# skypilot-org/skypilot

Hardware: AMD Instinct MI355X
Metric: tokens/sec (node) sky-launched Llama-3-8B (higher is better)
Workload: dtype bf16; 1 GPU; model=llama3-8b, global_batch=6, seq_len=4096, parallelism=dp1, sky_launched=True

## Files before the change

### skypilot_amd/models/llama.py

```python
from __future__ import annotations

import math
from dataclasses import dataclass

import torch
import torch.nn as nn

from skypilot_amd import ops


@dataclass
class LlamaConfig:
    name: str = "llama3-8b"
    vocab_size: int = 128256
    hidden_size: int = 4096
    intermediate_size: int = 14336
    num_layers: int = 32
    num_heads: int = 32
    num_kv_heads: int = 8
    head_dim: int = 128
    rope_theta: float = 500000.0
    norm_eps: float = 1e-5
    max_seq_len: int = 8192
    tie_embeddings: bool = False
# ... 51 lines not shown
                                      i32(lens))
        cache.write_rows_fp8(attn.layer_idx, k, v, *infer_ctx.kv_write_idx)
        return
    for i, (slot, ln) in enumerate(zip(slots, lens)):
        cache.write_prefill(attn.layer_idx, slot, k[i:i + 1], v[i:i + 1], ln)


def append_attention(attn, q, k, v, infer_ctx):
    cache = infer_ctx.cache
    if cache.kv_dtype == "fp8":
        li = attn.layer_idx
        cache.write_rows_fp8(li, k, v, infer_ctx.append_slots,
                             infer_ctx.append_start, infer_ctx.append_lens)
        return ops.attn_append_fp8(q, cache.k[li], cache.v[li],
                                   cache.k_exp[li], cache.v_exp[li],
                                   infer_ctx.append_slots,
                                   infer_ctx.append_start,
                                   infer_ctx.append_lens, attn.scale)
    for i, (slot, start, ln) in enumerate(zip(infer_ctx.append_slots_l,
                                              infer_ctx.append_start_l,
                                              infer_ctx.append_lens_l)):
        cache.write_append(attn.layer_idx, slot, start, k[i:i + 1],
                           v[i:i + 1], ln)
    return ops.attn_append(q, cache.k[attn.layer_idx],
                           cache.v[attn.layer_idx], infer_ctx.append_slots,
                           infer_ctx.append_start, infer_ctx.append_lens,
                           attn.scale)


class Attention(nn.Module):
    def __init__(self, cfg: LlamaConfig):
        super().__init__()
        self.cfg = cfg
        h, d = cfg.hidden_size, cfg.head_dim
        self.n_q, self.n_kv = cfg.num_heads, cfg.num_kv_heads
        self.wq = nn.Linear(h, self.n_q * d, bias=cfg.attn_bias)
        self.wk = nn.Linear(h, self.n_kv * d, bias=cfg.attn_bias)
        self.wv = nn.Linear(h, self.n_kv * d, bias=cfg.attn_bias)
        self.wo = nn.Linear(self.n_q * d, h, bias=False)
        self.scale = 1.0 / math.sqrt(d)
        self._wqkv = None
        self._bqkv = None

    def packed_qkv(self):
        if self._wqkv is None:
            self._wqkv = torch.cat(
                [self.wq.weight, self.wk.weight, self.wv.weight],
                0).contiguous()
            if self.wq.bias is not None:
                self._bqkv = torch.cat(
                    [self.wq.bias, self.wk.bias, self.wv.bias],
                    0).contiguous()
        return self._wqkv

    def forward(self, x, cos, sin, positions, infer_ctx=None,
                qkv=None):
        d = self.cfg.head_dim
        if x is None:
            B, S = qkv.shape[0], 1
        else:
            B, S, _ = x.shape
        decode = infer_ctx is not None and infer_ctx.mode == "decode"
        if decode:
            cache = infer_ctx.cache
            if qkv is None:
                qkv = ops.decode_linear(x.reshape(B, -1),
                                        self.packed_qkv())
            qkv = qkv.reshape(B, -1)
            if self._bqkv is not None:
                qkv = qkv + self._bqkv
            li = self.layer_idx
            if cache.kv_dtype == "fp8":
                o = ops.attn_decode_qkv_fp8(
                    qkv, cache.k[li], cache.v[li], cache.k_exp[li],
                    cache.v_exp[li], cos, sin, positions, infer_ctx.kv_lens,
                    infer_ctx.slot_ids_i32, self.n_q, self.n_kv, self.scale)
            else:
                o = ops.attn_decode_qkv(
                    qkv, cache.k[li], cache.v[li], cos, sin, positions,
                    infer_ctx.kv_lens, infer_ctx.slot_ids_i32, self.n_q,
                    self.n_kv, self.scale)
            return ops.decode_linear(o.reshape(B, self.n_q * d),
                                     self.wo.weight).view(B, S, -1)
        lin = torch.nn.functional.linear
        q = lin(x, self.wq.weight, self.wq.bias).view(B, S, self.n_q, d)
        k = lin(x, self.wk.weight, self.wk.bias).view(B, S, self.n_kv, d)
        v = lin(x, self.wv.weight, self.wv.bias).view(B, S, self.n_kv, d)
        q = ops.rope(q.reshape(B * S, self.n_q, d), cos, sin,
                     positions).view(B, S, self.n_q, d)
        k = ops.rope(k.reshape(B * S, self.n_kv, d), cos, sin,
                     positions).view(B, S, self.n_kv, d)
        if infer_ctx is None:
            o = ops.attention(q, k, v, self.scale, causal=True)
        elif infer_ctx.mode == "append":
            o = append_attention(self, q, k, v, infer_ctx)
        else:
            prefill_cache_write(self, k, v, infer_ctx)
            o = ops.attention(q, k, v, self.scale, causal=True)
        return lin(o.reshape(B, S, self.n_q * d), self.wo.weight)


class MLP(nn.Module):
    def __init__(self, cfg: LlamaConfig):
        super().__init__()
        h, m = cfg.hidden_size, cfg.intermediate_size
        self.w_gate_up = nn.Linear(h, 2 * m, bias=False)
        self.w_down = nn.Linear(m, h, bias=False)
        self.m = m

    def forward(self, x, infer_ctx=None):
        decode = infer_ctx is not None and infer_ctx.mode == "decode"
        lin = ops.decode_linear if decode else torch.nn.functional.linear
        return lin(ops.swiglu(lin(x, self.w_gate_up.weight)),
                   self.w_down.weight)

    def down_from_gu(self, gu):
        return ops.decode_linear(ops.swiglu(gu), self.w_down.weight)



class Block(nn.Module):
    def __init__(self, cfg: LlamaConfig, layer_idx: int):
        super().__init__()
        self.attn = Attention(cfg)
        self.attn.layer_idx = layer_idx
        self.mlp = MLP(cfg)
        self.attn_norm = nn.Parameter(torch.ones(cfg.hidden_size))
        self.mlp_norm = nn.Parameter(torch.ones(cfg.hidden_size))
        self.eps = cfg.norm_eps

    def forward(self, x, cos, sin, positions, infer_ctx=None):
        x = x + self.attn(ops.rmsnorm(x, self.attn_norm, self.eps), cos, sin,
                          positions, infer_ctx)
        x = x + self.mlp(ops.rmsnorm(x, self.mlp_norm, self.eps),
                         infer_ctx)
        return x


class Llama(nn.Module):
    def __init__(self, cfg: LlamaConfig):
        super().__init__()
        self.cfg = cfg
        self.embed = nn.Embedding(cfg.vocab_size, cfg.hidden_size)
        self.blocks = nn.ModuleList(
            Block(cfg, i) for i in range(cfg.num_layers))
        self.final_norm = nn.Parameter(torch.ones(cfg.hidden_size))
        self.lm_head = nn.Linear(cfg.hidden_size, cfg.vocab_size, bias=False)
        if cfg.tie_embeddings:
            self.lm_head.weight = self.embed.weight
        self._rope = None

    def _tables(self, device):
        if self._rope is None or self._rope[0].device != device:
            self._rope = rope_tables(self.cfg, device)
        return self._rope

    def forward(self, tokens: torch.Tensor, positions: torch.Tensor = None,
                infer_ctx=None) -> torch.Tensor:
        B, S = tokens.shape
        cos, sin = self._tables(tokens.device)
        if positions is None:
            positions = torch.arange(S, dtype=torch.int32,
                                     device=tokens.device)
            positions = positions.unsqueeze(0).expand(B, S).reshape(-1)
        x = self.embed(tokens)
        if infer_ctx is not None and infer_ctx.mode == "decode":
            res = None
            for blk in self.blocks:
                if not hasattr(blk.attn, "_wqkv"):
                    if res is None:
                        h = ops.rmsnorm(x, blk.attn_norm, blk.eps)
                    else:
                        x, h = ops.rmsnorm_res(x, res, blk.attn_norm,
                                               blk.eps)
                    a = blk.attn(h, cos, sin, positions, infer_ctx)
                    x, h2 = ops.rmsnorm_res(x, a, blk.mlp_norm, blk.eps)
                    res = blk.mlp(h2, infer_ctx)
                    continue
                x, qkv = ops.decode_norm_linear(
                    x, res, blk.attn_norm, blk.eps, blk.attn.packed_qkv())
                a = blk.attn(None, cos, sin, positions, infer_ctx,
                             qkv=qkv)
                x, gu = ops.decode_norm_linear(
                    x, a, blk.mlp_norm, blk.eps, blk.mlp.w_gate_up.weight)
                res = blk.mlp.down_from_gu(gu)
            _, logits = ops.decode_norm_linear(
                x, res, self.final_norm, self.cfg.norm_eps,
                self.lm_head.weight)
            return logits
        for blk in self.blocks:
            x = blk(x, cos, sin, positions, infer_ctx)
        if infer_ctx is not None and infer_ctx.mode == "append":
            last = (infer_ctx.append_lens.long() - 1).clamp(min=0)
            x = x[torch.arange(B, device=x.device), last].unsqueeze(1)
        x = ops.rmsnorm(x, self.final_norm, self.cfg.norm_eps)
# ... 29 lines not shown
```

### skypilot_amd/ops/__init__.py

```python
from __future__ import annotations

import importlib.util
import math
import os
from pathlib import Path

import torch

_C = None
_LOAD_ERR: Exception | None = None


def _load():
    global _C, _LOAD_ERR
    if _C is not None:
        return _C
    so = Path(__file__).resolve().parent / "_C.so"
    try:
        if not so.exists():
            raise ImportError(
                f"native extension {so} not built; run "
                "`python -m skypilot_amd.ops.build`")
        spec = importlib.util.spec_from_file_location("skypilot_amd.ops._C",
                                                      so)
# ... 162 lines not shown
        with torch.enable_grad():
            qd = q.detach().requires_grad_()
            kd = k.detach().requires_grad_()
            vd = v.detach().requires_grad_()
            out = attention_ref(qd, kd, vd, ctx.scale, ctx.causal)
            gq, gk, gv = torch.autograd.grad(out, (qd, kd, vd), dO)
        return gq, gk, gv, None, None


def attention(q, k, v, scale=None, causal=True):
    if scale is None:
        scale = 1.0 / math.sqrt(q.shape[-1])
    return _AttentionFn.apply(q, k, v, scale, causal)


class _CrossEntropyFn(torch.autograd.Function):

    @staticmethod
    def forward(ctx, logits, targets, ignore_index):
        if logits.is_cuda:
            C = _require_native("cross_entropy")
            n_valid = int((targets != ignore_index).sum().item())
            n_valid = max(n_valid, 1)
            logits = logits.contiguous()
            loss = C.cross_entropy_fused(logits, targets.int(),
                                         1.0 / n_valid, ignore_index)
            ctx.save_for_backward(logits)
            ctx.native = True
            return loss.sum() / n_valid
        ctx.native = False
        ctx.save_for_backward(logits, targets)
        ctx.ignore_index = ignore_index
        return cross_entropy_ref(logits, targets, ignore_index)

    @staticmethod
    def backward(ctx, g):
        if ctx.native:
            (dlogits,) = ctx.saved_tensors
            if not (isinstance(g, torch.Tensor) and g.numel() == 1
                    and float(g) == 1.0):
                dlogits = dlogits * g
            return dlogits, None, None
        logits, targets = ctx.saved_tensors
        with torch.enable_grad():
            ld = logits.detach().requires_grad_()
            loss = cross_entropy_ref(ld, targets, ctx.ignore_index)
            (gl,) = torch.autograd.grad(loss, (ld,), g)
        return gl, None, None


def fused_cross_entropy(logits, targets, ignore_index: int = -100):
    return _CrossEntropyFn.apply(logits, targets, ignore_index)


class _SwiGLUFn(torch.autograd.Function):
    @staticmethod
    def forward(ctx, gu):
        ctx.save_for_backward(gu)
        if gu.is_cuda:
            C = _require_native("swiglu")
            return C.swiglu_fwd(gu.contiguous())
        M = gu.shape[-1] // 2
        g, u = gu.float().split(M, dim=-1)
        return (torch.nn.functional.silu(g) * u).to(gu.dtype)

    @staticmethod
    def backward(ctx, dy):
        (gu,) = ctx.saved_tensors
        if gu.is_cuda:
            C = native()
            return C.swiglu_bwd(gu.contiguous(), dy.contiguous())
        M = gu.shape[-1] // 2
        g, u = gu.float().split(M, dim=-1)
        dyf = dy.float()
        sg = torch.sigmoid(g)
        silu = g * sg
        dg = dyf * u * (sg + silu * (1 - sg))
        du = dyf * silu
        return torch.cat([dg, du], dim=-1).to(gu.dtype)


def swiglu(gu):
    return _SwiGLUFn.apply(gu)


def attn_decode_ref(q, kc, vc, kv_lens, slot_ids, scale):
    B, Hq, D = q.shape
    Hkv = kc.shape[2]
    rep = Hq // Hkv
    out = torch.empty_like(q)
    for i in range(B):
        slot = int(slot_ids[i])
        L = int(kv_lens[i])
        k = kc[slot, :L].float()
        v = vc[slot, :L].float()
        kf = k.repeat_interleave(rep, dim=1)
        vf = v.repeat_interleave(rep, dim=1)
        att = torch.einsum("hd,lhd->hl", q[i].float(), kf) * scale
        p = att.softmax(-1)
        out[i] = torch.einsum("hl,lhd->hd", p, vf).to(q.dtype)
    return out


def attn_decode(q, kc, vc, kv_lens, slot_ids, scale):
    if q.is_cuda:
        C = _require_native("attn_decode")
        return C.attn_decode(q.contiguous(), kc, vc, kv_lens.int(),
                             slot_ids.int(), scale)
    return attn_decode_ref(q, kc, vc, kv_lens, slot_ids, scale)


def attn_append_ref(q, kc, vc, slot_ids, q_start, q_lens, scale):
    n, Sq, Hq, D = q.shape
    S_max, Hkv = kc.shape[1], kc.shape[2]
    rep = Hq // Hkv
    out = torch.zeros_like(q)
    for b in range(n):
        slot, start, ln = int(slot_ids[b]), int(q_start[b]), int(q_lens[b])
        if ln == 0:
            continue
        L = min(start + ln, S_max)
        qf = q[b, :ln].float().permute(1, 0, 2)
        kf = kc[slot, :L].float().permute(1, 0, 2).repeat_interleave(
            rep, dim=0)
        vf = vc[slot, :L].float().permute(1, 0, 2).repeat_interleave(
            rep, dim=0)
        att = torch.matmul(qf, kf.transpose(-1, -2)) * scale
        pos = start + torch.arange(ln, device=q.device)
        mask = torch.arange(L, device=q.device)[None, :] > pos[:, None]
        p = att.masked_fill(mask, float("-inf")).softmax(-1)
        out[b, :ln] = torch.matmul(p, vf).permute(1, 0, 2).to(q.dtype)
    return out


def attn_append(q, kc, vc, slot_ids, q_start, q_lens, scale):
    if q.is_cuda:
        C = _require_native("attn_append")
        return C.attn_append(q.contiguous(), kc, vc, slot_ids, q_start,
                             q_lens, scale)
    return attn_append_ref(q, kc, vc, slot_ids, q_start, q_lens, scale)


def kv_quantize(x: torch.Tensor):
    xf = x.detach().float()
    amax = xf.abs().amax(-1)
    u = amax.contiguous().view(torch.int32) & 0x7FFFFFFF
    n = (u >> 23) - 135 + ((u & 0x7FFFFF) > 0x600000).to(torch.int32)
    n = n.clamp(-126, 127)
    n = torch.where(u == 0, torch.zeros_like(n), n)
    inv = ((127 - n).clamp(min=1) << 23).view(torch.float32)
    codes = (xf * inv.unsqueeze(-1)).to(torch.float8_e4m3fn).view(torch.uint8)
    return codes.contiguous(), (n + 127).to(torch.uint8)


def kv_dequantize(codes: torch.Tensor, exp: torch.Tensor) -> torch.Tensor:
    scale = (exp.to(torch.int32) << 23).view(torch.float32)
    return codes.view(torch.float8_e4m3fn).float() * scale.unsqueeze(-1)


def kv_write_fp8(k, v, kc, vc, ke, ve, slot_ids, starts, lens):
    if k.is_cuda:
        C = _require_native("kv_write_fp8")
        C.kv_write_fp8(k.contiguous(), v.contiguous(), kc, vc, ke, ve,
                       slot_ids, starts, lens)
        return
    n, S = k.shape[0], k.shape[1]
# ... 248 lines not shown
    blk = torch.empty(6, n, dtype=torch.int32)
    blk[0] = rowvec(temperature, torch.float32).contiguous().view(torch.int32)
    blk[1] = rowvec(top_p, torch.float32).contiguous().view(torch.int32)
    blk[2] = rowvec(clamp_k(top_k), torch.int64).clamp(
        0, 2 ** 31 - 1).to(torch.int32)
    blk[3] = (sd & _M32).to(torch.int32)
    blk[4] = (sd >> 32).to(torch.int32)
    blk[5] = rowvec(wrap32(counter), torch.int64).to(torch.int32)
    return blk


def sample_tokens_reference(logits, temperature, top_p, top_k, seed,
                            counter):
    logits = logits.reshape(-1, logits.shape[-1])
    n = logits.shape[0]
    blk = pack_samp(n, temperature, top_p, top_k, seed, counter)
    Ts = blk[0].view(torch.float32).tolist()
    ps = blk[1].view(torch.float32).tolist()
    ks = blk[2].tolist()
    los, his, cs = blk[3].tolist(), blk[4].tolist(), blk[5].tolist()
    toks, taus = [], []
    for i in range(n):
        sd = ((his[i] & _M32) << 32) | (los[i] & _M32)
        r = sample_row_reference(logits[i], Ts[i], ps[i], ks[i], sd, cs[i])
        toks.append(r["token"])
        taus.append(r["tau"])
    return (torch.tensor(toks, dtype=torch.long),
            torch.tensor(taus, dtype=torch.float32))


def sample_tokens(logits, temperature, top_p, top_k, seed, counter):
    if not logits.is_cuda:
        return sample_tokens_reference(logits, temperature, top_p, top_k,
                                       seed, counter)
    C = _require_native("sample_tokens")
    if logits.dtype != torch.bfloat16 or logits.dim() != 2:
        raise ValueError("sample_tokens: logits must be bf16 [n, V] on GPU")
    n = logits.shape[0]
    blk = pack_samp(n, temperature, top_p, top_k, seed,
                    counter).to(logits.device)
    toks, tau = C.sample_tokens(logits.contiguous(), blk[:5], blk[5])
    return toks, tau


def decode_sample_advance(logits, stage, ring, ctr, samp):
    C = _require_native("decode_sample_advance")
    C.decode_sample_advance(logits.contiguous(), stage, ring, ctr, samp)


def decode_swiglu_down(gu, weight):
    return decode_linear(swiglu(gu), weight)


def attn_decode_qkv(qkv, kc, vc, cos, sin, positions, kv_lens, slot_ids,
                    Hq, Hkv, scale):
    D = kc.shape[3]
    if qkv.is_cuda and qkv.dtype == torch.bfloat16 and D == 128:
        C = _require_native("attn_decode_qkv")
        return C.attn_decode_qkv(qkv.contiguous(), kc, vc, cos, sin,
                                 positions.int(), kv_lens.int(),
                                 slot_ids.int(), Hq, Hkv, scale)
    q = rope_kvwrite(qkv, kc, vc, cos, sin, positions, slot_ids, Hq, Hkv)
    return attn_decode(q, kc, vc, kv_lens, slot_ids, scale)


def rope_kvwrite(qkv, kc, vc, cos, sin, positions, slot_ids, Hq, Hkv):
    D = kc.shape[3]
    n = qkv.shape[0]
    if qkv.is_cuda and qkv.dtype == torch.bfloat16 and D == 128:
        C = _require_native("rope_kvwrite")
        return C.rope_kvwrite(qkv.contiguous(), kc, vc, cos, sin,
                              positions.int(), slot_ids.int(), Hq, Hkv)
    q, k, v = qkv.split([Hq * D, Hkv * D, Hkv * D], dim=-1)
    qr = rope(q.reshape(n, Hq, D), cos, sin, positions)
    kr = rope(k.reshape(n, Hkv, D), cos, sin, positions)
    pos = positions.long()
    kc[slot_ids.long(), pos] = kr
    vc[slot_ids.long(), pos] = v.reshape(n, Hkv, D)
    return qr


__all__ = [
    "rmsnorm", "rope", "attention", "fused_cross_entropy", "attn_decode",
    "swiglu", "decode_linear", "rmsnorm_res", "rope_kvwrite",
    "decode_swiglu_down",
    "native", "native_available", "rmsnorm_ref", "rope_ref",
    "attention_ref", "cross_entropy_ref", "attn_decode_ref",
    "attn_append", "attn_append_ref",
    "kv_quantize", "kv_dequantize", "kv_write_fp8", "attn_decode_qkv_fp8",
    "attn_append_fp8", "attn_decode_fp8",
]
```

### skypilot_amd/ops/csrc/bindings.cpp

```cpp
#include <torch/extension.h>

#include <ATen/hip/HIPContext.h>
#include <hip/hip_runtime.h>

#include <limits>
#include <vector>

#include "attn_append.h"
#include "attn_launch.h"
#include "kv_fp8_launch.h"

#define CHECK_GPU(x) TORCH_CHECK(x.is_cuda(), #x " must be on GPU")
#define CHECK_CONTIG(x) TORCH_CHECK(x.is_contiguous(), #x " must be contiguous")
#define CHECK_BF16(x) \
  TORCH_CHECK(x.scalar_type() == at::kBFloat16, #x " must be bf16")

static hipStream_t cur_stream() {
  return at::hip::getCurrentHIPStream().stream();
}

extern "C" {
void rmsnorm_fwd_launch(const void*, const void*, void*, float*, long long,
                        int, float, hipStream_t);
void rmsnorm_bwd_launch(const void*, const void*, const void*, const float*,
// ... 550 lines not shown
        (float)scale, cur_stream());
  return O;
}

static void check_fp8_weight(const char* op, const torch::Tensor& W8,
                             const torch::Tensor& scale, int64_t I,
                             const torch::Tensor& first) {
  TORCH_CHECK(W8.defined() && (W8.scalar_type() == at::kByte ||
                               W8.scalar_type() == at::kFloat8_e4m3fn),
              op, ": W8 must be uint8 or float8_e4m3fn, got ",
              W8.scalar_type());
  check_dense(op, "W8", W8, W8.scalar_type(), first);
  TORCH_CHECK(W8.dim() == 2 && W8.size(1) == I, op,
              ": W8 must be [O, I] with I = ", I, ", got ", W8.sizes());
  TORCH_CHECK(W8.size(0) >= 1 &&
                  W8.size(0) <= std::numeric_limits<int>::max(),
              op, ": W8 must have at least one row, got ", W8.sizes());
  check_dense(op, "scale", scale, at::kFloat, first);
  TORCH_CHECK(scale.numel() == W8.size(0), op, ": scale must have O = ",
              W8.size(0), " elements, got ", scale.numel());
}

std::vector<torch::Tensor> skinny_gemm_fp8_norm(
    torch::Tensor x, torch::Tensor res, torch::Tensor nw, double eps,
    torch::Tensor W8, torch::Tensor scale, bool want_xout) {
  const char* op = "skinny_gemm_fp8_norm";
  check_dense(op, "x", x, at::kBFloat16, x);
  TORCH_CHECK(x.dim() == 2, op, ": x must be [N, I], got ", x.sizes());
  const int N = (int)x.size(0), I = (int)x.size(1);
  TORCH_CHECK(I >= 1024 && I <= 4096 && I % 1024 == 0, op,
              ": I must be 1024, 2048, 3072 or 4096, got ", I);
  TORCH_CHECK(N >= 1 && N <= 2, op, ": N must be 1 or 2, got ", N);
  check_fp8_weight(op, W8, scale, I, x);
  const int O = (int)W8.size(0);
  TORCH_CHECK(O % 2 == 0, op, ": O must be even, got ", O);
  check_dense(op, "nw", nw, at::kBFloat16, x);
  TORCH_CHECK(nw.numel() == I, op, ": nw must have I = ", I,
              " elements, got ", nw.numel());
  const bool has_res = res.defined() && res.numel() > 0;
  if (has_res) {
    check_dense(op, "res", res, at::kBFloat16, x);
    TORCH_CHECK(res.sizes() == x.sizes(), op, ": res must be empty or have "
                "x's shape ", x.sizes(), ", got ", res.sizes());
  }
  auto y = torch::empty({N, O}, x.options());
  torch::Tensor xout;
  if (want_xout) xout = torch::empty_like(x);
  skinny_gemm_fp8_norm_launch(
      W8.data_ptr(), scale.data_ptr<float>(), x.data_ptr(),
      has_res ? res.data_ptr() : nullptr, nw.data_ptr(),
      want_xout ? xout.data_ptr() : nullptr, (float)eps, y.data_ptr(),
      N, I, O, cur_stream());
  if (!want_xout) xout = x;
  return {xout, y};
}

void adamw_step_mt(torch::Tensor ptrs, torch::Tensor wd_arr,
                   torch::Tensor sizes, torch::Tensor chunk_tensor,
                   torch::Tensor chunk_start, double lr, double beta1,
                   double beta2, double eps, int64_t step,
                   double grad_scale) {
  CHECK_GPU(ptrs); CHECK_GPU(chunk_tensor);
  adamw_mt_launch(ptrs.data_ptr(), wd_arr.data_ptr(), sizes.data_ptr(),
                  chunk_tensor.data_ptr(), chunk_start.data_ptr(),
                  (long long)chunk_tensor.numel(), (float)lr, (float)beta1,
                  (float)beta2, (float)eps, (int)step, (float)grad_scale,
                  cur_stream());
}

torch::Tensor skinny_gemm_swiglu(torch::Tensor GU, torch::Tensor W) {
  CHECK_GPU(GU); CHECK_CONTIG(GU); CHECK_BF16(GU);
  CHECK_GPU(W); CHECK_CONTIG(W); CHECK_BF16(W);
  const int N = (int)GU.size(0), M = (int)GU.size(1) / 2;
  const int O = (int)W.size(0);
  TORCH_CHECK(W.size(1) == M, "skinny_gemm_swiglu: dims mismatch");
  TORCH_CHECK(N >= 1 && N <= 4, "skinny_gemm_swiglu: N must be 1..4");
  TORCH_CHECK(M % 512 == 0, "skinny_gemm_swiglu: M %% 512 != 0");
  auto y = torch::empty({N, O}, GU.options());
  skinny_gemm_swiglu_launch(W.data_ptr(), GU.data_ptr(), y.data_ptr(), N,
                            M, O, cur_stream());
  return y;
}

torch::Tensor transpose_bf16(torch::Tensor X) {
  CHECK_GPU(X); CHECK_CONTIG(X); CHECK_BF16(X);
  int R = X.size(0), C = X.size(1);
  TORCH_CHECK(R % 64 == 0 && C % 64 == 0, "transpose_bf16: dims % 64");
  auto Y = torch::empty({C, R}, X.options());
  transpose_bf16_launch(X.data_ptr(), Y.data_ptr(), R, C, cur_stream());
  return Y;
}

torch::Tensor gemm_nt(torch::Tensor A, torch::Tensor B) {
  CHECK_GPU(A); CHECK_CONTIG(A); CHECK_BF16(A);
  CHECK_GPU(B); CHECK_CONTIG(B); CHECK_BF16(B);
  long long M = A.size(1);
  int I = A.size(0), J = B.size(0);
  TORCH_CHECK(B.size(1) == M, "gemm_nt: inner dims mismatch");
  TORCH_CHECK(M % 64 == 0, "gemm_nt: M % 64 != 0");
  TORCH_CHECK(I % 128 == 0 && J % 256 == 0, "gemm_nt: I%128/J%256");
  auto C = torch::empty({I, J}, A.options());
  gemm_nt_launch(A.data_ptr(), B.data_ptr(), C.data_ptr(), I, J, M,
                 cur_stream());
  return C;
}

torch::Tensor wgrad_tn(torch::Tensor dy, torch::Tensor x) {
  CHECK_GPU(dy); CHECK_CONTIG(dy); CHECK_BF16(dy);
  CHECK_GPU(x); CHECK_CONTIG(x); CHECK_BF16(x);
  long long M = dy.size(0);
  int I = dy.size(1), J = x.size(1);
  TORCH_CHECK(x.size(0) == M, "wgrad_tn: token dims mismatch");
  auto dyT = transpose_bf16(dy);
  auto xT = transpose_bf16(x);
  return gemm_nt(dyT, xT);
}

torch::Tensor skinny_gemm_fp8(torch::Tensor X, torch::Tensor W8,
                              torch::Tensor scale) {
  const char* op = "skinny_gemm_fp8";
  check_dense(op, "X", X, at::kBFloat16, X);
  TORCH_CHECK(X.dim() == 2, op, ": X must be [N, I], got ", X.sizes());
  const int64_t N = X.size(0), I = X.size(1);
  TORCH_CHECK(N >= 1 && N <= 8, op, ": N must be 1..8, got ", N);
  TORCH_CHECK(I >= 16 && I % 16 == 0 &&
                  I <= std::numeric_limits<int>::max(),
              op, ": I must be a positive multiple of 16, got ", I);
  check_fp8_weight(op, W8, scale, I, X);
  const int64_t O = W8.size(0);
  auto y = torch::empty({N, O}, X.options());
  skinny_gemm_fp8_launch(W8.data_ptr(), scale.data_ptr<float>(),
                         X.data_ptr(), y.data_ptr(), (int)N, (int)I, (int)O,
                         cur_stream());
  return y;
}

torch::Tensor skinny_gemm(torch::Tensor X, torch::Tensor W) {
  CHECK_GPU(X); CHECK_CONTIG(X); CHECK_BF16(X);
  CHECK_GPU(W); CHECK_CONTIG(W); CHECK_BF16(W);
  const int N = (int)X.size(0), I = (int)X.size(1), O = (int)W.size(0);
  TORCH_CHECK(W.size(1) == I, "skinny_gemm: inner dims mismatch");
  TORCH_CHECK(N >= 1 && N <= 8, "skinny_gemm: N must be 1..8");
  TORCH_CHECK(I % 512 == 0, "skinny_gemm: I must be a multiple of 512");
  auto y = torch::empty({N, O}, X.options());
  skinny_gemm_launch(W.data_ptr(), X.data_ptr(), y.data_ptr(), N, I, O,
                     cur_stream());
  return y;
}

std::vector<torch::Tensor> rmsnorm_res(torch::Tensor x, torch::Tensor res,
                                       torch::Tensor w, double eps) {
  const char* op = "rmsnorm_res";
  check_dense(op, "x", x, at::kBFloat16, x);
  TORCH_CHECK(x.dim() >= 1, op, ": x must be [..., H], got a scalar");
  const int64_t H = x.size(-1);
  TORCH_CHECK(H >= 256 && H % 256 == 0 && H <= 8192, op,
              ": H must be a multiple of 256 and <= 8192, got ", H);
  check_dense(op, "res", res, at::kBFloat16, x);
  TORCH_CHECK(res.sizes() == x.sizes(), op, ": res must have x's shape ",
              x.sizes(), ", got ", res.sizes());
  check_dense(op, "w", w, at::kBFloat16, x);
  TORCH_CHECK(w.numel() == H, op, ": w must have H = ", H,
              " elements, got ", w.numel());
  const int64_t rows = x.numel() / H;
  TORCH_CHECK(rows <= std::numeric_limits<int>::max(), op, ": ", rows,
              " rows exceed the grid limit 2^31 - 1");
  auto x_out = torch::empty_like(x);
  auto h_out = torch::empty_like(x);
  if (rows > 0)
    rmsnorm_res_launch(x.data_ptr(), res.data_ptr(), w.data_ptr(),
                       x_out.data_ptr(), h_out.data_ptr(), (int)rows, (int)H,
                       (float)eps, cur_stream());
  return {x_out, h_out};
}

void decode_advance(torch::Tensor logits, torch::Tensor stage,
                    torch::Tensor ring, torch::Tensor ctr) {
  const char* op = "decode_advance";
  check_dense(op, "logits", logits, at::kBFloat16, logits);
  TORCH_CHECK(logits.dim() >= 1, op,
              ": logits must be [b, V], got a scalar");
  const int64_t V = logits.size(-1);
  TORCH_CHECK(V >= 1 && V <= std::numeric_limits<int>::max(), op,
              ": V must be in [1, 2^31 - 1], got ", V);
  const int64_t b = logits.numel() / V;
  check_dense(op, "stage", stage, at::kInt, logits);
  TORCH_CHECK(stage.dim() == 2 && stage.size(0) == 6 && stage.size(1) == b,
              op, ": stage must be [6, b] = [6, ", b, "], got ",
              stage.sizes());
  check_dense(op, "ring", ring, at::kLong, logits);
  TORCH_CHECK(ring.dim() == 2 && ring.size(0) >= 1 &&
                  ring.size(0) <= std::numeric_limits<int>::max() &&
                  ring.size(1) == b,
              op, ": ring must be [chunk >= 1, b] = [chunk, ", b, "], got ",
              ring.sizes());
  check_dense(op, "ctr", ctr, at::kLong, logits);
  TORCH_CHECK(ctr.numel() == 1, op, ": ctr must hold one element, got ",
              ctr.sizes());
// ... 94 lines not shown
}

torch::Tensor swiglu_fwd(torch::Tensor gu) {
  CHECK_GPU(gu); CHECK_CONTIG(gu); CHECK_BF16(gu);
  const int M2 = (int)gu.size(-1);
  TORCH_CHECK(M2 % 16 == 0, "swiglu_fwd: last dim must be 2*M with "
              "M % 8 == 0, got ", M2);
  long long rows = gu.numel() / M2;
  auto sizes = gu.sizes().vec();
  sizes.back() = M2 / 2;
  auto y = torch::empty(sizes, gu.options());
  swiglu_fwd_launch(gu.data_ptr(), y.data_ptr(), rows, M2 / 2,
                    cur_stream());
  return y;
}

torch::Tensor swiglu_bwd(torch::Tensor gu, torch::Tensor dy) {
  CHECK_GPU(gu); CHECK_CONTIG(gu); CHECK_BF16(gu);
  CHECK_GPU(dy); CHECK_CONTIG(dy); CHECK_BF16(dy);
  const int M2 = (int)gu.size(-1);
  TORCH_CHECK(M2 % 16 == 0, "swiglu_bwd: last dim must be 2*M with "
              "M % 8 == 0, got ", M2);
  auto ysizes = gu.sizes().vec();
  ysizes.back() = M2 / 2;
  TORCH_CHECK(dy.sizes() == at::IntArrayRef(ysizes),
              "swiglu_bwd: dy must have the shape of swiglu_fwd(gu)");
  long long rows = gu.numel() / M2;
  auto dgu = torch::empty_like(gu);
  swiglu_bwd_launch(gu.data_ptr(), dy.data_ptr(), dgu.data_ptr(), rows,
                    M2 / 2, cur_stream());
  return dgu;
}

torch::Tensor mfma_probe(torch::Tensor A, torch::Tensor B) {
  CHECK_GPU(A); CHECK_BF16(A); CHECK_CONTIG(A); CHECK_CONTIG(B);
  TORCH_CHECK(A.size(0) == 16 && A.size(1) == 32);
  TORCH_CHECK(B.size(0) == 32 && B.size(1) == 16);
  auto C = torch::zeros({16, 16}, A.options().dtype(at::kFloat));
  mfma_probe_launch(A.data_ptr(), B.data_ptr(), C.data_ptr<float>(),
                    cur_stream());
  return C;
}

torch::Tensor mfma32_probe(torch::Tensor A, torch::Tensor B) {
  CHECK_GPU(A); CHECK_BF16(A); CHECK_CONTIG(A); CHECK_CONTIG(B);
  TORCH_CHECK(A.size(0) == 32 && A.size(1) == 16);
  TORCH_CHECK(B.size(0) == 16 && B.size(1) == 32);
  auto C = torch::zeros({32, 32}, A.options().dtype(at::kFloat));
  mfma32_probe_launch(A.data_ptr(), B.data_ptr(), C.data_ptr<float>(),
                      cur_stream());
  return C;
}

torch::Tensor trb16_probe(int64_t mode, torch::Tensor ref_dev) {
  auto out = torch::zeros({64, 4}, ref_dev.options().dtype(at::kFloat));
  trb16_probe_launch(out.data_ptr<float>(), (int)mode, cur_stream());
  return out;
}

torch::Tensor permlane_probe(torch::Tensor ref_dev) {
  auto out = torch::zeros({64, 2}, ref_dev.options().dtype(at::kFloat));
  permlane_probe_launch(out.data_ptr<float>(), cur_stream());
  return out;
}

PYBIND11_MODULE(TORCH_EXTENSION_NAME, m) {
  m.def("rmsnorm_fwd", &rmsnorm_fwd);
  m.def("rmsnorm_bwd", &rmsnorm_bwd);
  m.def("rope", &rope);
  m.def("adamw_step", &adamw_step);
  m.def("cross_entropy_fused", &cross_entropy_fused);
  m.def("attn_fwd", &attn_fwd);
  m.def("attn_bwd", &attn_bwd, py::arg("Q"), py::arg("K"), py::arg("V"),
        py::arg("O"), py::arg("dO"), py::arg("lse"), py::arg("scale"),
        py::arg("causal"), py::arg("dkv_variant") = -1,
        py::arg("dq_variant") = -1);
  m.def("attn_decode", &attn_decode);
  m.def("attn_append", &attn_append);
  m.def("skinny_gemm", &skinny_gemm);
  m.def("skinny_gemm_fp8", &skinny_gemm_fp8);
  m.def("transpose_bf16", &transpose_bf16);
  m.def("gemm_nt", &gemm_nt);
  m.def("wgrad_tn", &wgrad_tn);
  m.def("adamw_step_mt", &adamw_step_mt);
  m.def("skinny_gemm_swiglu", &skinny_gemm_swiglu);
  m.def("rmsnorm_res", &rmsnorm_res);
  m.def("rope_kvwrite", &rope_kvwrite);
  m.def("decode_advance", &decode_advance);
  m.def("sample_tokens", &sample_tokens);
  m.def("decode_sample_advance", &decode_sample_advance);
  m.def("attn_decode_qkv", &attn_decode_qkv);
  m.def("kv_write_fp8", &kv_write_fp8);
  m.def("attn_decode_qkv_fp8", &attn_decode_qkv_fp8);
  m.def("attn_append_fp8", &attn_append_fp8);
  m.def("skinny_gemm_fp8_norm", &skinny_gemm_fp8_norm);
  m.def("swiglu_fwd", &swiglu_fwd);
  m.def("swiglu_bwd", &swiglu_bwd);
  m.def("mfma_probe", &mfma_probe);
  m.def("mfma32_probe", &mfma32_probe);
  m.def("trb16_probe", &trb16_probe);
  m.def("permlane_probe", &permlane_probe);
}
```

### skypilot_amd/ops/csrc/wgrad_gemm.hip

```cpp
#include <cstdlib>

#include "common.h"

typedef __attribute__((ext_vector_type(16))) float f32x16;
#define MFMA32W(a, b, c) \
  __builtin_amdgcn_mfma_f32_32x32x16_bf16(a, b, c, 0, 0, 0)

#define TP 72
extern "C" __global__ __launch_bounds__(256) void transpose_bf16_kernel(
    const unsigned short* __restrict__ in, unsigned short* __restrict__ out,
    int R, int C) {
  __shared__ unsigned short t[64 * TP];
  const int tiles_r = R >> 6;
  const int tiles_c = C >> 6;
  const int tid = threadIdx.x;
  for (long long tile = blockIdx.x; tile < (long long)tiles_r * tiles_c;
       tile += gridDim.x) {
    const int tr = (int)(tile / tiles_c);
    const int tc = (int)(tile % tiles_c);
    const long long r0 = (long long)tr << 6;
    const long long c0 = (long long)tc << 6;
    __syncthreads();
#pragma unroll
    for (int i = 0; i < 2; ++i) {
      int r = (tid >> 3) + 32 * i;
      int c8 = (tid & 7) * 8;
      *(s16x8*)&t[r * TP + c8] =
          *(const s16x8*)(in + (r0 + r) * C + c0 + c8);
    }
    __syncthreads();
#pragma unroll
    for (int i = 0; i < 2; ++i) {
      int c = (tid >> 3) + 32 * i;
      int r8 = (tid & 7) * 8;
      s16x8 v;
#pragma unroll
      for (int j = 0; j < 8; ++j) v[j] = t[(r8 + j) * TP + c];
      *(s16x8*)(out + (c0 + c) * R + r0 + r8) = v;
    }
  }
}

__device__ __forceinline__ void gload_lds16w(const void* g, void* l) {
  __builtin_amdgcn_global_load_lds(
      (const __attribute__((address_space(1))) unsigned int*)g,
      (__attribute__((address_space(3))) unsigned int*)l, 16, 0, 0);
}

template <int BM>
__global__ __launch_bounds__(512, 1) void gemm_nt_kernel(
    const unsigned short* __restrict__ A, const unsigned short* __restrict__ B,
    unsigned short* __restrict__ C, int I, int J, long long M,
    int swz_grid) {
  __shared__ unsigned short a_lds[2][BM * 64];
  __shared__ unsigned short b_lds[2][256 * 64];

  constexpr int MT = BM / 64;
  const int tid = threadIdx.x;
  const int lane = tid & 63;
  const int w = tid >> 6;
  const int wm = w >> 2;
  const int wn = w & 3;
  const int col = lane & 31;
  const int h = lane >> 5;

  int bid = blockIdx.x;
  if (swz_grid) {
    const int nwg = gridDim.x;
    const int q = nwg >> 3, r = nwg & 7;
    const int xcd = bid & 7, off = bid >> 3;
    bid = (xcd < r ? xcd * (q + 1) : r * (q + 1) + (xcd - r) * q) + off;
  }
  const int nbj = J >> 8;
  const int bi = bid / nbj;
  const int bj = bid % nbj;
  const long long i0 = (long long)bi * BM;
  const long long j0 = (long long)bj << 8;

  f32x16 acc[MT][2];
#pragma unroll
  for (int it = 0; it < MT; ++it)
#pragma unroll
    for (int jt = 0; jt < 2; ++jt)
#pragma unroll
      for (int r = 0; r < 16; ++r) acc[it][jt][r] = 0.f;

  const int srow = lane >> 3;
  const int schk = lane & 7;
#define WG_STAGE_A(bufi, kt)                                              \
  {                                                                       \
    _Pragma("unroll") for (int ii = 0; ii < BM / 64; ++ii) {              \
      int r0 = (w * (BM / 64) + ii) * 8;                                  \
      int row = r0 + srow;                                                \
      gload_lds16w(                                                       \
          A + (i0 + row) * M + (long long)(kt) * 64 +                     \
              ((schk ^ (row & 7)) << 3),                                  \
          (char*)a_lds[bufi] + r0 * 128);                                 \
    }                                                                     \
  }
#define WG_STAGE_B(bufi, kt)                                              \
  {                                                                       \
    _Pragma("unroll") for (int ii = 0; ii < 4; ++ii) {                    \
      int r0 = (w * 4 + ii) * 8;                                          \
      int row = r0 + srow;                                                \
      gload_lds16w(                                                       \
          B + (j0 + row) * M + (long long)(kt) * 64 +                     \
              ((schk ^ (row & 7)) << 3),                                  \
          (char*)b_lds[bufi] + r0 * 128);                                 \
    }                                                                     \
  }

  const int n_kt = (int)(M >> 6);
  WG_STAGE_A(0, 0);
  WG_STAGE_B(0, 0);
  asm volatile("s_waitcnt vmcnt(0)" ::: "memory");
  __builtin_amdgcn_s_barrier();

  for (int kt = 0; kt < n_kt; ++kt) {
    const int buf = kt & 1;
    const bool more = kt + 1 < n_kt;
#pragma unroll
    for (int ks = 0; ks < 4; ++ks) {
      s16x8 af[MT], bf[2];
      const int chk = (2 * ks + h) << 4;
#pragma unroll
      for (int it = 0; it < MT; ++it) {
        int row = wm * (BM / 2) + it * 32 + col;
        af[it] = *(const s16x8*)(
            (char*)a_lds[buf] + row * 128 + (chk ^ ((row & 7) << 4)));
      }
#pragma unroll
      for (int jt = 0; jt < 2; ++jt) {
        int row = wn * 64 + jt * 32 + col;
        bf[jt] = *(const s16x8*)(
            (char*)b_lds[buf] + row * 128 + (chk ^ ((row & 7) << 4)));
      }
      if (more) {
        if (ks == 0) WG_STAGE_A(buf ^ 1, kt + 1);
        if (ks == 1) WG_STAGE_B(buf ^ 1, kt + 1);
      }
      __builtin_amdgcn_s_barrier();
      asm volatile("s_waitcnt lgkmcnt(0)" ::: "memory");
      __builtin_amdgcn_sched_barrier(0);
      __builtin_amdgcn_s_setprio(1);
#pragma unroll
      for (int it = 0; it < MT; ++it)
#pragma unroll
        for (int jt = 0; jt < 2; ++jt)
          acc[it][jt] =
              MFMA32W(as_bf16x8(af[it]), as_bf16x8(bf[jt]), acc[it][jt]);
      __builtin_amdgcn_s_setprio(0);
      if (ks == 3) asm volatile("s_waitcnt vmcnt(0)" ::: "memory");
      __builtin_amdgcn_s_barrier();
    }
  }

#pragma unroll
  for (int it = 0; it < MT; ++it) {
    const long long ib = i0 + wm * (BM / 2) + it * 32;
#pragma unroll
    for (int jt = 0; jt < 2; ++jt) {
      const long long jb = j0 + wn * 64 + jt * 32;
#pragma unroll
      for (int r = 0; r < 16; ++r) {
        long long irow = ib + (r & 3) + ((r >> 2) << 3) + (h << 2);
        C[irow * J + jb + col] = f2bf(acc[it][jt][r]);
      }
    }
  }
}

extern "C" void transpose_bf16_launch(const void* in, void* out, int R,
                                      int C, hipStream_t stream) {
  long long tiles = ((long long)R >> 6) * (C >> 6);
  int grid = tiles > 4096 ? 4096 : (int)tiles;
  hipLaunchKernelGGL(transpose_bf16_kernel, dim3(grid), dim3(256), 0,
                     stream, (const unsigned short*)in,
                     (unsigned short*)out, R, C);
}

extern "C" void gemm_nt_launch(const void* A, const void* B, void* C, int I,
                               int J, long long M, hipStream_t stream) {
  const long long blocks256 = ((long long)I >> 8) * (J >> 8);
  if (I % 256 == 0 && blocks256 >= 512) {
    dim3 grid((unsigned)blocks256);
    hipLaunchKernelGGL(gemm_nt_kernel<256>, grid, dim3(512), 0, stream,
                       (const unsigned short*)A, (const unsigned short*)B,
                       (unsigned short*)C, I, J, M, 1);
  } else {
    dim3 grid((unsigned)(((long long)I >> 7) * (J >> 8)));
    hipLaunchKernelGGL(gemm_nt_kernel<128>, grid, dim3(512), 0, stream,
                       (const unsigned short*)A, (const unsigned short*)B,
                       (unsigned short*)C, I, J, M, 1);
  }
}
```

Before: 21700 tokens/s.

## Route linear weight-grads through transposed GEMM paths and pack QKV backward

Adds custom autograd linear and fused QKV linear ops whose backward computes the weight gradient through a native routine. For large token counts and specific shapes (gate_up, down), that routine pre-transposes dy (and optionally x) so the library GEMM sees a more favorable layout. The QKV backward concatenates the three grads so dx and dW each take one GEMM instead of three. The bf16 transpose kernel is rewritten to use 64-thread blocks, register-level byte permutes and an XOR-swizzled LDS tile, replacing the padded scalar-gather version. The extra transposes and concatenations add memory traffic, and the gain depends on the library GEMM being faster on the transposed layout.

```diff
diff --git a/skypilot_amd/models/llama.py b/skypilot_amd/models/llama.py
--- a/skypilot_amd/models/llama.py
+++ b/skypilot_amd/models/llama.py
@@ -157,10 +157,12 @@
                     self.n_kv, self.scale)
             return ops.decode_linear(o.reshape(B, self.n_q * d),
                                      self.wo.weight).view(B, S, -1)
-        lin = torch.nn.functional.linear
-        q = lin(x, self.wq.weight, self.wq.bias).view(B, S, self.n_q, d)
-        k = lin(x, self.wk.weight, self.wk.bias).view(B, S, self.n_kv, d)
-        v = lin(x, self.wv.weight, self.wv.bias).view(B, S, self.n_kv, d)
+        q, k, v = ops.qkv_linear(x, self.wq.weight, self.wk.weight,
+                                 self.wv.weight, self.wq.bias, self.wk.bias,
+                                 self.wv.bias)
+        q = q.view(B, S, self.n_q, d)
+        k = k.view(B, S, self.n_kv, d)
+        v = v.view(B, S, self.n_kv, d)
         q = ops.rope(q.reshape(B * S, self.n_q, d), cos, sin,
                      positions).view(B, S, self.n_q, d)
         k = ops.rope(k.reshape(B * S, self.n_kv, d), cos, sin,
@@ -172,7 +174,7 @@
         else:
             prefill_cache_write(self, k, v, infer_ctx)
             o = ops.attention(q, k, v, self.scale, causal=True)
-        return lin(o.reshape(B, S, self.n_q * d), self.wo.weight)
+        return ops.linear(o.reshape(B, S, self.n_q * d), self.wo.weight)
 
 
 class MLP(nn.Module):
@@ -185,7 +187,7 @@
 
     def forward(self, x, infer_ctx=None):
         decode = infer_ctx is not None and infer_ctx.mode == "decode"
-        lin = ops.decode_linear if decode else torch.nn.functional.linear
+        lin = ops.decode_linear if decode else ops.linear
         return lin(ops.swiglu(lin(x, self.w_gate_up.weight)),
                    self.w_down.weight)
 
diff --git a/skypilot_amd/ops/__init__.py b/skypilot_amd/ops/__init__.py
--- a/skypilot_amd/ops/__init__.py
+++ b/skypilot_amd/ops/__init__.py
@@ -268,6 +268,77 @@
 
 def swiglu(gu):
     return _SwiGLUFn.apply(gu)
+
+
+def _rows(t):
+    return t.reshape(-1, t.shape[-1])
+
+
+class _LinearFn(torch.autograd.Function):
+    @staticmethod
+    def forward(ctx, x, w, b, route):
+        ctx.save_for_backward(x, w)
+        ctx.route = route
+        return torch.nn.functional.linear(x, w, b)
+
+    @staticmethod
+    def backward(ctx, dy):
+        x, w = ctx.saved_tensors
+        dy2 = _rows(dy)
+        dx = dw = db = None
+        if ctx.needs_input_grad[0]:
+            dx = (dy2 @ w).view(x.shape)
+        if ctx.needs_input_grad[1]:
+            dw = native().linear_wgrad(dy2.contiguous(),
+                                       _rows(x).contiguous(), ctx.route)
+        if ctx.needs_input_grad[2]:
+            db = dy2.sum(0)
+        return dx, dw, db, None
+
+
+def linear(x, w, b=None, route: int = -1):
+    if not (x.is_cuda and x.dtype == torch.bfloat16
+            and w.dtype == torch.bfloat16):
+        return torch.nn.functional.linear(x, w, b)
+    _require_native("linear")
+    return _LinearFn.apply(x, w, b, route)
+
+
+class _QKVLinearFn(torch.autograd.Function):
+    @staticmethod
+    def forward(ctx, x, wq, wk, wv, bq, bk, bv, route):
+        ctx.save_for_backward(x, wq, wk, wv)
+        ctx.route = route
+        lin = torch.nn.functional.linear
+        return lin(x, wq, bq), lin(x, wk, bk), lin(x, wv, bv)
+
+    @staticmethod
+    def backward(ctx, dq, dk, dv):
+        x, wq, wk, wv = ctx.saved_tensors
+        outs = [wq.shape[0], wk.shape[0], wv.shape[0]]
+        dy = torch.cat([_rows(dq), _rows(dk), _rows(dv)], dim=1)
+        need = ctx.needs_input_grad
+        dx = None
+        if need[0]:
+            dx = (dy @ torch.cat([wq, wk, wv], dim=0)).view(x.shape)
+        dws = [None, None, None]
+        if need[1] or need[2] or need[3]:
+            dws = native().linear_wgrad(dy, _rows(x).contiguous(),
+                                        ctx.route).split(outs, dim=0)
+        dbs = [None, None, None]
+        if need[4] or need[5] or need[6]:
+            dbs = [d if need[4 + i] else None
+                   for i, d in enumerate(dy.sum(0).split(outs))]
+        return (dx, *dws, *dbs, None)
+
+
+def qkv_linear(x, wq, wk, wv, bq=None, bk=None, bv=None, route: int = -1):
+    lin = torch.nn.functional.linear
+    if not (x.is_cuda and x.dtype == torch.bfloat16
+            and wq.dtype == torch.bfloat16):
+        return lin(x, wq, bq), lin(x, wk, bk), lin(x, wv, bv)
+    _require_native("qkv_linear")
+    return _QKVLinearFn.apply(x, wq, wk, wv, bq, bk, bv, route)
 
 
 def attn_decode_ref(q, kc, vc, kv_lens, slot_ids, scale):
@@ -682,7 +753,8 @@
 
 __all__ = [
     "rmsnorm", "rope", "attention", "fused_cross_entropy", "attn_decode",
-    "swiglu", "decode_linear", "rmsnorm_res", "rope_kvwrite",
+    "swiglu", "linear", "qkv_linear",
+    "decode_linear", "rmsnorm_res", "rope_kvwrite",
     "decode_swiglu_down",
     "native", "native_available", "rmsnorm_ref", "rope_ref",
     "attention_ref", "cross_entropy_ref", "attn_decode_ref",
diff --git a/skypilot_amd/ops/csrc/bindings.cpp b/skypilot_amd/ops/csrc/bindings.cpp
--- a/skypilot_amd/ops/csrc/bindings.cpp
+++ b/skypilot_amd/ops/csrc/bindings.cpp
@@ -656,13 +656,53 @@
   return y;
 }
 
+static bool tile_dims(const torch::Tensor& X) {
+  return X.size(0) > 0 && X.size(1) > 0 && X.size(0) % 64 == 0 &&
+         X.size(1) % 64 == 0 &&
+         X.size(0) <= std::numeric_limits<int>::max() &&
+         X.size(1) <= std::numeric_limits<int>::max();
+}
+static bool aligned16(const torch::Tensor& X) {
+  return reinterpret_cast<uintptr_t>(X.data_ptr()) % 16 == 0;
+}
+static bool transposable(const torch::Tensor& X) {
+  return tile_dims(X) && aligned16(X);
+}
+
+static void check_transpose_arg(const char* op, const char* name,
+                                const torch::Tensor& X,
+                                const torch::Tensor& first) {
+  check_dense(op, name, X, at::kBFloat16, first);
+  TORCH_CHECK(X.dim() == 2, op, ": ", name, " must be 2-D, got ", X.sizes());
+  TORCH_CHECK(aligned16(X), op, ": ", name, " must start on a 16-byte "
+              "boundary (storage offset ", X.storage_offset(), ")");
+}
+
+static void check_transpose_src(const char* op, const char* name,
+                                const torch::Tensor& X,
+                                const torch::Tensor& first) {
+  check_transpose_arg(op, name, X, first);
+  TORCH_CHECK(tile_dims(X), op, ": ", name, " dims must be positive "
+              "multiples of 64 (dims % 64), got ", X.sizes());
+}
+
 torch::Tensor transpose_bf16(torch::Tensor X) {
-  CHECK_GPU(X); CHECK_CONTIG(X); CHECK_BF16(X);
+  check_transpose_src("transpose_bf16", "X", X, X);
   int R = X.size(0), C = X.size(1);
-  TORCH_CHECK(R % 64 == 0 && C % 64 == 0, "transpose_bf16: dims % 64");
   auto Y = torch::empty({C, R}, X.options());
   transpose_bf16_launch(X.data_ptr(), Y.data_ptr(), R, C, cur_stream());
   return Y;
+}
+
+void transpose_bf16_out(torch::Tensor X, torch::Tensor Y) {
+  const char* op = "transpose_bf16_out";
+  check_transpose_src(op, "X", X, X);
+  check_transpose_arg(op, "Y", Y, X);
+  TORCH_CHECK(Y.size(0) == X.size(1) &&
+              Y.size(1) == X.size(0), op, ": Y must be [", X.size(1), ", ",
+              X.size(0), "] for X ", X.sizes(), ", got ", Y.sizes());
+  transpose_bf16_launch(X.data_ptr(), Y.data_ptr(), (int)X.size(0),
+                        (int)X.size(1), cur_stream());
 }
 
 torch::Tensor gemm_nt(torch::Tensor A, torch::Tensor B) {
@@ -688,6 +728,69 @@
   auto dyT = transpose_bf16(dy);
   auto xT = transpose_bf16(x);
   return gemm_nt(dyT, xT);
+}
+
+struct WgradRoute {
+  int64_t out, in;
+  int route;
+};
+static const WgradRoute kWgradRoutes[] = {
+    {28672, 4096, 1},
+    {4096, 14336, 2},
+};
+static const int64_t kWgradMinTokens = 8192;
+
+static int wgrad_table_route(int64_t M, int64_t out, int64_t in) {
+  if (M < kWgradMinTokens) return 0;
+  for (const auto& r : kWgradRoutes)
+    if (r.out == out && r.in == in) return r.route;
+  return 0;
+}
+
+std::vector<torch::Tensor> linear_wgrad_packed(std::vector<torch::Tensor> dys,
+                                               torch::Tensor x,
+                                               int64_t route) {
+  const char* op = "linear_wgrad";
+  TORCH_CHECK(route >= -1 && route <= 2, op, ": route must be -1 (table), "
+              "0 (library), 1 (both transposed) or 2 (dy transposed), got ",
+              route);
+  TORCH_CHECK(!dys.empty(), op, ": needs at least one dy");
+  check_dense(op, "x", x, at::kBFloat16, x);
+  TORCH_CHECK(x.dim() == 2, op, ": x must be [M, in], got ", x.sizes());
+  const int64_t M = x.size(0), in = x.size(1);
+  int64_t total = 0;
+  bool tiles = transposable(x);
+  for (const auto& dy : dys) {
+    check_dense(op, "dy", dy, at::kBFloat16, x);
+    TORCH_CHECK(dy.dim() == 2 && dy.size(0) == M, op, ": dy must be [M = ",
+                M, ", out], got ", dy.sizes());
+    total += dy.size(1);
+    tiles = tiles && transposable(dy);
+  }
+  if (route < 0) route = wgrad_table_route(M, total, in);
+  std::vector<torch::Tensor> dWs;
+  if (route == 0 || !tiles) {
+    for (const auto& dy : dys) dWs.push_back(at::mm(dy.t(), x));
+    return dWs;
+  }
+  auto dyT = at::empty({total, M}, x.options());
+  int64_t off = 0;
+  for (const auto& dy : dys) {
+    transpose_bf16_out(dy, dyT.narrow(0, off, dy.size(1)));
+    off += dy.size(1);
+  }
+  auto dW = route == 1 ? at::linear(dyT, transpose_bf16(x)) : at::mm(dyT, x);
+  if (dys.size() == 1) return {dW};
+  off = 0;
+  for (const auto& dy : dys) {
+    dWs.push_back(dW.narrow(0, off, dy.size(1)));
+    off += dy.size(1);
+  }
+  return dWs;
+}
+
+torch::Tensor linear_wgrad(torch::Tensor dy, torch::Tensor x, int64_t route) {
+  return linear_wgrad_packed({dy}, x, route)[0];
 }
 
 torch::Tensor skinny_gemm_fp8(torch::Tensor X, torch::Tensor W8,
@@ -948,6 +1051,11 @@
   m.def("transpose_bf16", &transpose_bf16);
   m.def("gemm_nt", &gemm_nt);
   m.def("wgrad_tn", &wgrad_tn);
+  m.def("transpose_bf16_out", &transpose_bf16_out);
+  m.def("linear_wgrad", &linear_wgrad, py::arg("dy"), py::arg("x"),
+        py::arg("route") = -1);
+  m.def("linear_wgrad_packed", &linear_wgrad_packed, py::arg("dys"),
+        py::arg("x"), py::arg("route") = -1);
   m.def("adamw_step_mt", &adamw_step_mt);
   m.def("skinny_gemm_swiglu", &skinny_gemm_swiglu);
   m.def("rmsnorm_res", &rmsnorm_res);
diff --git a/skypilot_amd/ops/csrc/wgrad_gemm.hip b/skypilot_amd/ops/csrc/wgrad_gemm.hip
--- a/skypilot_amd/ops/csrc/wgrad_gemm.hip
+++ b/skypilot_amd/ops/csrc/wgrad_gemm.hip
@@ -6,37 +6,41 @@
 #define MFMA32W(a, b, c) \
   __builtin_amdgcn_mfma_f32_32x32x16_bf16(a, b, c, 0, 0, 0)
 
-#define TP 72
-extern "C" __global__ __launch_bounds__(256) void transpose_bf16_kernel(
+typedef __attribute__((ext_vector_type(4))) unsigned int u32x4;
+extern "C" __global__ __launch_bounds__(64) void transpose_bf16_kernel(
     const unsigned short* __restrict__ in, unsigned short* __restrict__ out,
     int R, int C) {
-  __shared__ unsigned short t[64 * TP];
+  __shared__ u32x4 t[64 * 8];
   const int tiles_r = R >> 6;
   const int tiles_c = C >> 6;
-  const int tid = threadIdx.x;
+  const int g = threadIdx.x >> 3;
+  const int s = threadIdx.x & 7;
   for (long long tile = blockIdx.x; tile < (long long)tiles_r * tiles_c;
        tile += gridDim.x) {
     const int tr = (int)(tile / tiles_c);
     const int tc = (int)(tile % tiles_c);
     const long long r0 = (long long)tr << 6;
     const long long c0 = (long long)tc << 6;
+    u32x4 v[8];
+#pragma unroll
+    for (int j = 0; j < 8; ++j)
+      v[j] = *(const u32x4*)(in + (r0 + 8 * g + j) * C + c0 + 8 * s);
     __syncthreads();
 #pragma unroll
-    for (int i = 0; i < 2; ++i) {
-      int r = (tid >> 3) + 32 * i;
-      int c8 = (tid & 7) * 8;
-      *(s16x8*)&t[r * TP + c8] =
-          *(const s16x8*)(in + (r0 + r) * C + c0 + c8);
+    for (int i = 0; i < 8; ++i) {
+      const unsigned sel = (i & 1) ? 0x07060302u : 0x05040100u;
+      u32x4 o;
+#pragma unroll
+      for (int m = 0; m < 4; ++m)
+        o[m] = __builtin_amdgcn_perm(v[2 * m + 1][i >> 1], v[2 * m][i >> 1],
+                                     sel);
+      t[(8 * s + i) * 8 + (g ^ s)] = o;
     }
     __syncthreads();
 #pragma unroll
-    for (int i = 0; i < 2; ++i) {
-      int c = (tid >> 3) + 32 * i;
-      int r8 = (tid & 7) * 8;
-      s16x8 v;
-#pragma unroll
-      for (int j = 0; j < 8; ++j) v[j] = t[(r8 + j) * TP + c];
-      *(s16x8*)(out + (c0 + c) * R + r0 + r8) = v;
+    for (int i = 0; i < 8; ++i) {
+      const int c = g + 8 * i;
+      *(u32x4*)(out + (c0 + c) * R + r0 + 8 * s) = t[c * 8 + (s ^ i)];
     }
   }
 }
@@ -174,7 +178,7 @@
                                       int C, hipStream_t stream) {
   long long tiles = ((long long)R >> 6) * (C >> 6);
   int grid = tiles > 4096 ? 4096 : (int)tiles;
-  hipLaunchKernelGGL(transpose_bf16_kernel, dim3(grid), dim3(256), 0,
+  hipLaunchKernelGGL(transpose_bf16_kernel, dim3(grid), dim3(64), 0,
                      stream, (const unsigned short*)in,
                      (unsigned short*)out, R, C);
 }
```

Result: faster. 22210 tokens/s (median of 6 runs) (+2.4%).
